# lucanest/Phyloformer

Measured on AMD Instinct MI355X. Metric: alignments/sec, 60-leaf/500-site LG+GC-like MSAs, Phyloformer forward (pf.ckpt), higher is better.
Workload: dtype f16x3-split MFMA (two fp16 limbs per operand, 3 passes), fp32 accumulate/residual

## Files before the change

phyloformer_amd/csrc/pf_device.hip.h:

```cpp
#pragma once
#include <hip/hip_runtime.h>
#include <stdint.h>

#include "pf_layout.h"

namespace pfk {

typedef float f32x4 __attribute__((ext_vector_type(4)));
typedef float f32x16 __attribute__((ext_vector_type(16)));
#if PF_F16
typedef _Float16 h16_t;
#define PF_MFMA(a, b, c) __builtin_amdgcn_mfma_f32_32x32x16_f16((a), (b), (c), 0, 0, 0)
#define PF_DOT2C "v_dot2c_f32_f16"
#define PF_CVT_PK "v_cvt_pk_f16_f32"
#define PF_NEG1_LO 0x0000bc00u
#define PF_NEG1_HI 0xbc000000u
#else
typedef __bf16 h16_t;
#define PF_MFMA(a, b, c) __builtin_amdgcn_mfma_f32_32x32x16_bf16((a), (b), (c), 0, 0, 0)
#define PF_DOT2C "v_dot2c_f32_bf16"
#define PF_CVT_PK "v_cvt_pk_bf16_f32"
#define PF_NEG1_LO 0x0000bf80u
#define PF_NEG1_HI 0xbf800000u
#endif
// ... 1084 lines not shown
        for (int q = 0; q < 8; ++q) v[q] = k + q < nparts ? sp[k + q] : 0.f;
#pragma unroll
        for (int q = 0; q < 8; ++q) acc += v[q];
    }
    out[pr] = acc * (wst ? wst[(size_t)(pr / P) * 4 + 1] : inv_L_total);
}

__global__ void __launch_bounds__(64) k_main_plan(const int* ucount, int* plan, int B, int P, int Lloc, int mode) {
    const int lane = threadIdx.x;
    int* const flist = plan + 4;
    int* const slist = flist + B;
    int* const cpre = slist + B;
    int nf = 0, ns = 0, tiles = 0;
    for (int b0 = 0; b0 < B; b0 += 64) {
        const int b = b0 + lane;
        const int K = b < B ? ucount[b] : 0;
        const bool split = b < B && main_dedup_split(K, Lloc, mode);
        const bool fused = b < B && !split;
        const unsigned long long ms = __ballot(split), mf = __ballot(fused), below = (1ull << lane) - 1ull;
        int incl = split ? compact_tiles(P, K) : 0;
        const int mine = incl;
#pragma unroll
        for (int d = 1; d < 64; d <<= 1) { const int o = __shfl_up(incl, d); if (lane >= d) incl += o; }
        if (split) { const int i = ns + __popcll(ms & below); slist[i] = b; cpre[i] = tiles + incl - mine; }
        if (fused) flist[nf + __popcll(mf & below)] = b;
        ns += __popcll(ms);
        nf += __popcll(mf);
        tiles += __shfl(incl, 63);
    }
    if (lane == 0) { plan[0] = nf; plan[1] = ns; plan[2] = tiles; plan[3] = 0; cpre[ns] = tiles; }
}

template <bool FLAT>
__global__ void __launch_bounds__(256) k_head_parts(MainArgs a) {
    const int ns = *a.acount;
    if (ns == 0) return;
    const int lane = threadIdx.x & 63, t = lane & 31;
    const int ntiles = (a.Lloc + 31) >> 5;
    const int ntasks = ns * a.nt_aln;
    for (int task = blockIdx.x * 4 + (threadIdx.x >> 6); task < ntasks; task += gridDim.x * 4) {
        const TilePos cur = tile_pos<FLAT, ROUTE_LIST>(a, task, ntiles);
        const LanePos lp = lane_pos<FLAT, ROUTE_LIST>(a, cur, t);
        const size_t row0 = ((size_t)cur.b * a.P + cur.r0 + (lp.in_r1 ? 1 : 0)) * a.Lloc;
        const float spz = a.term[row0 + a.srep[(size_t)cur.b * a.Lloc + lp.l]];
        const bool straddle = lp.wrap < 32;
        const long slot0 = (long)cur.b * a.slots_aln + cur.kt + (FLAT ? cur.r0 : 0);
        for (int part = 0; part < (straddle ? 2 : 1); ++part) {
            const float so = half32_sum((lp.valid && lp.in_r1 == (part == 1)) ? spz : 0.f);
            if (lane == 0) a.outpart[slot0 + part] = so;
        }
    }
}

struct SiteClassArgs {
    const uint8_t* idx;
    int* srep;
    int* ulist;
    int* ucount;
    int N, Lloc, dedup;
};
constexpr int SC_THREADS = 1024, SC_MAX_SITES = 4096;
__global__ void __launch_bounds__(SC_THREADS) k_site_classes(SiteClassArgs a) {
    __shared__ __attribute__((aligned(16))) uint32_t hsh[SC_MAX_SITES];
    __shared__ int wsum[SC_THREADS / 64];
    const int b = blockIdx.x, tid = threadIdx.x, lane = tid & 63, wave = tid >> 6;
    const uint8_t* ib = a.idx + (size_t)b * a.N * a.Lloc;
    int* const srep = a.srep + (size_t)b * a.Lloc;
    int* const ulist = a.ulist + (size_t)b * a.Lloc;
    const bool dedup = a.dedup && a.Lloc <= SC_MAX_SITES;
    auto same_column = [&](int c, int l) {
        unsigned diff = 0;
#pragma unroll 8
        for (int n = 0; n < a.N; ++n) diff |= (unsigned)(ib[(size_t)n * a.Lloc + c] ^ ib[(size_t)n * a.Lloc + l]);
        return diff == 0;
    };
    if (dedup) {
        for (int l = tid; l < a.Lloc; l += SC_THREADS) {
            uint32_t hv = 0x811C9DC5u;
#pragma unroll 8
            for (int n = 0; n < a.N; ++n) hv = (hv ^ ib[(size_t)n * a.Lloc + l]) * 0x01000193u;
            hsh[l] = hv;
        }
        __syncthreads();
    }
    int base = 0;
    for (int l0 = 0; l0 < a.Lloc; l0 += SC_THREADS) {
        const int l = l0 + tid;
        int rep = l;
        if (dedup && l < a.Lloc) {
            const uint32_t mine = hsh[l];
            int cand = l;
            for (int c0 = 0; c0 < l && cand == l; c0 += 4) {
                const u32x4 v = *reinterpret_cast<const u32x4*>(hsh + c0);
#pragma unroll
                for (int i = 3; i >= 0; --i)
                    if (v[i] == mine && c0 + i < l) cand = c0 + i;
            }
            if (cand < l) {
                if (same_column(cand, l)) rep = cand;
                else
                    for (int c = cand + 1; c < l && rep == l; ++c)
                        if (hsh[c] == mine && same_column(c, l)) rep = c;
            }
        }
        const bool first = l < a.Lloc && rep == l;
        if (l < a.Lloc) srep[l] = rep;
        const unsigned long long m = __ballot(first);
        if (lane == 0) wsum[wave] = __popcll(m);
        __syncthreads();
        int before = 0, total = 0;
#pragma unroll
        for (int w = 0; w < SC_THREADS / 64; ++w) { const int n = wsum[w]; total += n; if (w < wave) before += n; }
        if (first) ulist[base + before + __popcll(m & ((1ull << lane) - 1ull))] = l;
        base += total;
// ... 434 lines not shown
```

phyloformer_amd/csrc/pf_layout.h:

```cpp
#pragma once

#ifndef PF_F16
#define PF_F16 1
#endif

namespace pfk {

constexpr int E = 64;
constexpr int NH = 4;
constexpr int HD = 16;
constexpr int FF = 256;
constexpr int NA = 22;
constexpr int SROW = 72;
constexpr int MROW = 4 * 64;
constexpr float LN_EPS = 1e-5f;

constexpr int FRAG_W1 = 0;
constexpr int FRAG_W2 = FRAG_W1 + 8 * 4 * 2 * 64;
constexpr int FRAG_WO = FRAG_W2 + 2 * 16 * 2 * 64;
constexpr int FRAG_WV = FRAG_WO + 2 * 4 * 2 * 64;
constexpr int FRAG_QK = FRAG_WV + 2 * 4 * 64;
#ifndef PF_WVLO_LDS
#define PF_WVLO_LDS 4
#endif
constexpr int WVLO_LDS = PF_WVLO_LDS;
constexpr int FRAG_WVLO = FRAG_QK + 4 * 2 * 16;
constexpr int FRAG_END = FRAG_WVLO + WVLO_LDS * 64;
constexpr int FRAG_U = FRAG_WV;
constexpr int U_FRAGS = FF * 4 / 16;
static_assert(FRAG_U + U_FRAGS <= FRAG_END, "the folded head fits the last block's tail");
constexpr int WVLO_FRAGS = 2 * 4 * 64;
constexpr int CONST_B1 = 0, CONST_B2 = 256, CONST_BQK = 320, CONST_HW = 328, CONST_HB = 392,
              CONST_C0 = 393, CONST_BOC = 400;
constexpr int CONST_LEN = 464;
constexpr int MAIN_LDS_BYTES = FRAG_END * 16 + CONST_LEN * 4;
constexpr int MFRAG_PER_PAIR = 2 * 2 * 32;

constexpr int MAIN_THREADS = 512;
constexpr int MAIN_WAVES = MAIN_THREADS / 64;

constexpr int PAIRTAB_ROWS = 22 * 22, PAIRTAB_W = 72;

#if defined(__HIPCC__)
#define PF_HD __host__ __device__
#else
#define PF_HD
#endif
#ifndef PF_MAIN_DEDUP_NUM
#define PF_MAIN_DEDUP_NUM 17
#define PF_MAIN_DEDUP_DEN 20
#endif
constexpr int MAIN_DEDUP_NUM = PF_MAIN_DEDUP_NUM, MAIN_DEDUP_DEN = PF_MAIN_DEDUP_DEN;
PF_HD inline bool main_dedup_split(int K, int L, int mode) {
    return mode == 2 || (mode == 1 && (long)K * MAIN_DEDUP_DEN <= (long)L * MAIN_DEDUP_NUM);
}
PF_HD inline int compact_tiles(int P, int K) { return K >= 32 ? (int)(((long)P * K + 31) >> 5) : P; }
PF_HD inline int compact_nvalid(int P, int K, int kt) {
    const long left = K >= 32 ? (long)P * K - (long)kt * 32 : K;
    return left < 32 ? (int)left : 32;
}
PF_HD inline int compact_wrap(int P, int K, int r0, int u0) {
    return (K >= 32 && r0 + 1 < P && K - u0 < 32) ? K - u0 : 32;
}
struct CompactTile { int r0, u0, nvalid, wrap; };
PF_HD inline CompactTile compact_tile(int P, int K, int kt) {
    CompactTile c;
    if (K >= 32) { const long tok0 = (long)kt * 32; c.r0 = (int)(tok0 / K); c.u0 = (int)(tok0 - (long)c.r0 * K); }
    else { c.r0 = kt; c.u0 = 0; }
    c.nvalid = compact_nvalid(P, K, kt);
    c.wrap = compact_wrap(P, K, c.r0, c.u0);
    return c;
}
PF_HD inline void compact_next(int K, int* r0, int* u0) {
    if (K < 32) { ++*r0; return; }
    *u0 += 32;
    if (*u0 >= K) { *u0 -= K; ++*r0; }
}
PF_HD inline int main_plan_ints(int B) { return 4 + 3 * B + 1; }

}
```

phyloformer_amd/csrc/pf_lib.hip:

```cpp
#include <hip/hip_runtime.h>
#include <dlfcn.h>

#include <algorithm>
#include <cmath>
#include <cstdarg>
#include <cstdio>
#include <cstdlib>
#include <cstring>
#include <functional>
#include <map>
#include <mutex>
#include <string>
#include <type_traits>
#include <vector>

#include "../../include/phyloformer_amd.h"
#include "pf_device.hip.h"
#include "pf_mha.hip.h"
#include "pf_precise.hip.h"
#include "pf_generic.hip.h"
#include "pf_boot.hip.h"
#include "pf_sites.hip.h"
#include "pf_sitemap.hip.h"
#include "pf_sites_host.h"
// ... 119 lines not shown
    std::vector<pfp::FfnW> ffn;
};

struct GenericWeights {
    F64Ends ends;
    bool ready = false;
    std::vector<pfg::AttnW> row, col;
    std::vector<pfg::FfnW> ffn;
};

constexpr int64_t SUB_FLOATS_DEFAULT = (int64_t)1 << 22;

struct DeviceBuffer {
    void* p = nullptr; size_t cap = 0;
    explicit DeviceBuffer(std::vector<DeviceBuffer*>& all) { all.push_back(this); }
    DeviceBuffer(const DeviceBuffer&) = delete;
    int reserve(pf_handle* h, size_t bytes);
    void release() { if (p) hipFree(p); p = nullptr; cap = 0; }
};
template <class T> struct Buffer : DeviceBuffer {
    using DeviceBuffer::DeviceBuffer;
    operator T*() const { return static_cast<T*>(p); }
};

}

struct pf_handle {
    int device = 0;
    int n_blocks = 0;
    hipStream_t stream = nullptr;
    hipStream_t stream2 = nullptr;
    hipStream_t cur = nullptr;
    hipEvent_t ev_fork = nullptr, ev_join = nullptr;
    hipDeviceProp_t prop;
    std::string err;
    int64_t max_seqs = 200;
    bool profile = false;
    bool profile_main_only = false;
    bool debug_keep = false;
    int ablate = 0;
    unsigned long long* phase_prof = nullptr;
    bool phase_prof_last = false;
    bool head_fold = true;
    bool force_rccl = false;
    int64_t ws_limit_bytes = (int64_t)24 << 30;
    float* table = nullptr;
    float* pair_table = nullptr;
    bool embed_mfma = false;
    int colstats_fine = -1;
    bool colstats_ring = true;
    bool materialize_x0 = false;
    bool site_dedup = true;
    int main_dedup = 1;
    float* first_consts = nullptr;
    float* first_img = nullptr;
    std::vector<BlockDev> blk;
    std::vector<void*> owned;
    std::vector<DeviceBuffer*> buffers;
    int pair_n = -1;
    Buffer<int16_t> pair_i{buffers}, pair_j{buffers};
    Buffer<char> ws{buffers}, ws2{buffers};
    bool overlap = true;
    int reserve_cus = 8;
    Buffer<uint8_t> d_idx{buffers};
    Buffer<float> d_out{buffers};
    Buffer<uint8_t> d_rep{buffers};
    Buffer<int32_t> d_map{buffers};
    Buffer<float> d_smap{buffers}, d_se{buffers}, d_prof{buffers};
    Buffer<double> d_mpart{buffers};
    Buffer<char> d_sub{buffers};
    int64_t sub_floats = SUB_FLOATS_DEFAULT;
    pftile::Plan tiled_plan;
    pftile::Tables tiled_tab;
    Buffer<char> d_tiled_tab{buffers};
    Buffer<char> d_nj{buffers}, d_nj_io{buffers};
    int64_t nj_calls = 0;
    int64_t bionj_calls = 0;
    Buffer<char> d_delta_io{buffers};
    int64_t delta_calls = 0;
    bool delta_atomic = true;
    Buffer<char> d_fit{buffers}, d_fit_io{buffers};
    int64_t fit_calls = 0;
    int64_t fit_lds_bytes = pffit::LDS_MAX_BYTES;
    Buffer<char> d_ols{buffers}, d_ols_io{buffers};
    int64_t ols_calls = 0;
    Buffer<char> d_bme{buffers};
    Buffer<float> d_bme_preds{buffers};
    int64_t bme_calls = 0;
    int64_t spr_calls = 0;
    bool spr_pairs_simple = false;
    int64_t spr_step_cap = 0;
    Buffer<char> d_sup{buffers}, d_sup_io{buffers};
    Buffer<uint8_t> d_sup_bad{buffers};
    int64_t sup_calls = 0;
    int64_t transfer_calls = 0;
    Buffer<char> d_con{buffers}, d_con_io{buffers};
    int64_t con_calls = 0;
    Buffer<char> d_td{buffers}, d_td_io{buffers};
    int64_t td_calls = 0;
    Buffer<float> d_w{buffers}, d_wst{buffers}, d_wtab{buffers};
    void* comm[2] = {nullptr, nullptr};
    int rank = 0, world = 1;
    int64_t coll_calls = 0;
    bool sharded_call = false;
    bool reducing = false;
    bool two_streams = true;
// ... 291 lines not shown
int save_tap(pf_handle* h, const std::string& name, const float* dptr, size_t n) {
    std::vector<float>& v = h->taps[name];
    v.resize(n);
    HIPCHK(h, hipStreamSynchronize(h->cur));
    HIPCHK(h, hipMemcpy(v.data(), dptr, n * sizeof(float), hipMemcpyDeviceToHost));
    return PF_OK;
}

int allreduce(pf_handle* h, void* buf, size_t count, int dtype = NCCL_FLOAT) {
    if (!h->sharded_call) return PF_OK;
    if (h->world <= 1 && !h->comm[0]) return PF_OK;
    if (!h->comm[0]) return fail(h, PF_ESTATE, "sharded forward on %d ranks needs pf_comm_init", h->world);
    ProfScope ps(h, K_ALLREDUCE);
    void* comm = h->comm[(h->cur == h->stream2 && h->stream2) ? 1 : 0];
    ++h->coll_calls;
    int rc = g_rccl.AllReduce(buf, buf, count, dtype, NCCL_SUM, comm, h->cur);
    if (rc != 0)
        return fail(h, PF_ERCCL, "ncclAllReduce failed: %s",
                    g_rccl.GetErrorString ? g_rccl.GetErrorString(rc) : "?");
    return PF_OK;
}

enum { PLAIN = 0, SITEMAP = 1, WEIGHTED = 2 };
constexpr int HEAD_PARTS = MODE_STATS + 1;
struct MainKind { int mode, flavour = PLAIN, route = ROUTE_ALL; };
using MainKernel = void (*)(MainArgs);
struct MainRow { MainKind kind; bool flat; MainKernel fn; };
const std::vector<MainRow>& main_kernels();

MainKernel main_kernel(MainKind k, bool flat) {
    for (const MainRow& r : main_kernels())
        if (r.kind.mode == k.mode && r.kind.flavour == k.flavour && r.kind.route == k.route && r.flat == flat) return r.fn;
    return nullptr;
}

int persistent_grid(const pf_handle* h, long ntasks, int per_block, int per_cu) {
    const int cus = std::max(1, h->prop.multiProcessorCount - (h->reducing ? h->reserve_cus : 0));
    return (int)std::max<long>(1, std::min<long>((long)per_cu * cus, (ntasks + per_block - 1) / per_block));
}

int launch_main(pf_handle* h, MainKind kind, const MainArgs& a, bool timed) {
    const MainKernel fn = main_kernel(kind, kind.route == ROUTE_COMPACT || a.flat);
    if (!fn) return fail(h, PF_ESTATE, "no k_main for mode %d, flavour %d, route %d", kind.mode, kind.flavour, kind.route);
    const int grid = persistent_grid(h, (long)a.B * a.nt_aln, MAIN_WAVES, 1);
    ProfScope ps(h, kind.mode == MODE_FIRST ? K_EMBED : K_MAIN, timed);
    hipLaunchKernelGGL(fn, dim3(grid), dim3(MAIN_THREADS), MAIN_LDS_BYTES, h->cur, a);
    HIPCHK(h, hipGetLastError());
    return PF_OK;
}

struct MainPlan { const int *nf, *ns, *flist, *slist, *cpre; };
MainPlan main_plan(const int* plan, int B) { return {&plan[0], &plan[1], &plan[4], &plan[4 + B], &plan[4 + 2 * B]}; }

int launch_main_routed(pf_handle* h, int mode, const MainArgs& m, const MainPlan& p) {
    int rc;
    MainArgs f = m, c = m;
    f.acount = p.nf; f.alist = p.flist;
    if ((rc = launch_main(h, {mode, PLAIN, ROUTE_LIST}, f, false))) return rc;
    c.acount = p.ns; c.alist = p.slist; c.cpre = p.cpre;
    c.term = m.spart; c.prof = nullptr;
    if ((rc = launch_main(h, {mode, PLAIN, ROUTE_COMPACT}, c, false))) return rc;
    if (mode != MODE_LAST && mode != MODE_LAST_FOLD) return launch_main(h, {MODE_STATS, PLAIN, ROUTE_LIST}, c, false);
    hipLaunchKernelGGL(main_kernel({HEAD_PARTS, PLAIN, ROUTE_LIST}, m.flat != 0), dim3(persistent_grid(h, (long)m.B * m.nt_aln, 4, 8)),
                       dim3(256), 0, h->cur, c);
    HIPCHK(h, hipGetLastError());
    return PF_OK;
}

struct RowStats { const float* p; int nparts; int flat; };
struct ShardRun {
    Workspace w;
    const uint8_t* d_idx;
    float* d_out;
    int B, N, P, Lloc, L_total;
    TilePlan tp;
    hipStream_t stream;
    RowStats rs;
    float* d_smap = nullptr;
    const float* d_w = nullptr;
    const float* d_wst = nullptr;
    bool routed = false;
};

int zero_fill(pf_handle* h, float* p, size_t n) {
    HIPCHK(h, hipMemsetAsync(p, 0, n * sizeof(float), h->cur));
    return PF_OK;
}

MainArgs main_args(pf_handle* h, const ShardRun& r) {
    MainArgs m{};
    m.x = r.w.x; m.qrow = r.w.qrow; m.qcol = r.w.qcol;
    m.mfrag = reinterpret_cast<const frag_t*>(r.w.mfrag); m.rq = r.w.rq; m.ctx = r.w.ctx; m.spart = r.w.spart;
    m.outpart = r.w.outpart; m.table = h->table; m.idx = r.d_idx; m.pair_i = h->pair_i; m.pair_j = h->pair_j;
    m.B = r.B; m.N = r.N; m.P = r.P; m.Lloc = r.Lloc;
    m.flat = r.tp.flat; m.nt_aln = r.tp.nt_aln; m.slots_aln = r.tp.slots_aln;
    m.store_x_last = h->debug_keep ? 1 : 0;
    m.trash_tok = (size_t)r.B * r.P * r.Lloc;
    m.ablate = h->ablate;
    m.prof = h->phase_prof_last ? nullptr : h->phase_prof;
    m.w = r.d_w;
    m.srep = r.w.srep;
    m.ulist = r.w.ulist; m.ucount = r.w.ucount;
    return m;
}

bool x0_on_the_fly(const pf_handle* h) {
    return !h->materialize_x0 && !h->embed_mfma && h->n_blocks > 1;
}

bool routes_main(const pf_handle* h, const ShardRun& r) {
    return h->main_dedup != 0 && !r.d_smap && !r.d_w && x0_on_the_fly(h) && r.Lloc > 0;
}

ShardRun shard_run(const pf_handle* h, const uint8_t* d_idx, float* d_out, int B, int N, int Lloc, int L_total,
                   float* d_smap = nullptr, const float* d_w = nullptr, const float* d_wst = nullptr) {
    ShardRun r{};
    r.d_idx = d_idx; r.d_out = d_out; r.d_smap = d_smap; r.d_w = d_w; r.d_wst = d_wst;
    r.B = B; r.N = N; r.P = N * (N - 1) / 2; r.Lloc = Lloc; r.L_total = L_total;
    r.tp = tile_plan(h, r.P, Lloc); r.stream = h->stream; r.routed = routes_main(h, r);
    return r;
}

int launch_site_classes(pf_handle* h, const SiteClassArgs& a, int B, int* plan = nullptr, int P = 0) {
    if (!a.Lloc) return PF_OK;
    ProfScope ps(h, K_SITE_CLASSES);
    hipLaunchKernelGGL(k_site_classes, dim3(B), dim3(SC_THREADS), 0, h->cur, a);
    HIPCHK(h, hipGetLastError());
    if (!plan) return PF_OK;
    hipLaunchKernelGGL(k_main_plan, dim3(1), dim3(64), 0, h->cur, a.ucount, plan, B, P, a.Lloc, h->main_dedup);
    HIPCHK(h, hipGetLastError());
    return PF_OK;
}

int save_route_taps(pf_handle* h, const ShardRun& r) {
    if (!r.Lloc) return PF_OK;
    const size_t nsite = (size_t)r.B * r.Lloc;
    int rc;
    if ((rc = save_tap(h, "srep", reinterpret_cast<const float*>(r.w.srep), nsite))) return rc;
    if ((rc = save_tap(h, "ulist", reinterpret_cast<const float*>(r.w.ulist), nsite))) return rc;
    if ((rc = save_tap(h, "ucount", reinterpret_cast<const float*>(r.w.ucount), (size_t)r.B))) return rc;
    if (r.routed) return save_tap(h, "plan", reinterpret_cast<const float*>(r.w.plan), (size_t)main_plan_ints(r.B));
    h->taps.erase("plan");
    return PF_OK;
}

int phase_first(pf_handle* h, const ShardRun& r) {
    if (!r.Lloc) return zero_fill(h, r.w.srow, (size_t)r.B * r.P * SROW);
    int rc;
    if (h->embed_mfma) {
        MainArgs m = main_args(h, r);
        m.wimg = reinterpret_cast<const frag_t*>(h->first_img); m.consts = h->first_consts;
        m.wv_lo = reinterpret_cast<const frag_t*>(h->blk[0].wv_lo);
        if ((rc = launch_main(h, {MODE_FIRST}, m, true))) return rc;
    } else {
        float* x0 = (x0_on_the_fly(h) && !h->debug_keep) ? nullptr : r.w.x;
        EmbedArgs e{r.d_idx, h->pair_i, h->pair_j, h->pair_table, h->table, x0, r.w.qrow, r.w.srow,
                    r.B, r.N, r.P, r.Lloc, h->bad_idx_dev, r.d_w};
        const int ntasks = r.B * r.P, wpb = EMBED_THREADS / 64;
        const int grid = std::max(1, std::min(h->prop.multiProcessorCount, (ntasks + wpb - 1) / wpb));
        ProfScope ps(h, K_EMBED);
        if (r.d_w) hipLaunchKernelGGL(k_embed<true>, dim3(grid), dim3(EMBED_THREADS), EMBED_LDS_BYTES, h->cur, e);
        else hipLaunchKernelGGL(k_embed<false>, dim3(grid), dim3(EMBED_THREADS), EMBED_LDS_BYTES, h->cur, e);
        HIPCHK(h, hipGetLastError());
    }
    if (h->debug_keep) return save_tap(h, "x0", r.w.x, (size_t)r.B * r.P * r.Lloc * 64);
    return PF_OK;
}

int tiles_of(int Lloc) { return (Lloc + 31) / 32; }

int launch_rowsum(pf_handle* h, const ShardRun& r, RowStats* rs) {
    if (rs->p == r.w.srow) return PF_OK;
    const int n = r.B * r.P * SROW;
    if (!r.Lloc) { *rs = RowStats{r.w.srow, 1, 0}; return zero_fill(h, r.w.srow, n); }
    ProfScope ps(h, K_ROWFIN);
    hipLaunchKernelGGL(k_rowsum, dim3((n + 255) / 256), dim3(256), 0, h->cur, rs->p, r.w.srow, r.B * r.P, rs->nparts,
                       rs->flat, r.P, r.Lloc, r.tp.slots_aln);
    HIPCHK(h, hipGetLastError());
    *rs = RowStats{r.w.srow, 1, 0};
    return PF_OK;
}

// ... 55 lines not shown
template <int MODE, bool FLAT, int FLAVOUR = PLAIN, int ROUTE = ROUTE_ALL>
MainRow main_row() { return {{MODE, FLAVOUR, ROUTE}, FLAT, k_main<MODE, FLAT, FLAVOUR == SITEMAP, FLAVOUR == WEIGHTED, ROUTE>}; }
template <bool FLAT>
MainRow head_parts_row() { return {{HEAD_PARTS, PLAIN, ROUTE_LIST}, FLAT, k_head_parts<FLAT>}; }
const std::vector<MainRow>& main_kernels() {
    static const std::vector<MainRow> rows = {
        main_row<MODE_MID0, true, PLAIN, ROUTE_LIST>(), main_row<MODE_MID0, false, PLAIN, ROUTE_LIST>(), main_row<MODE_MID0, true, PLAIN, ROUTE_COMPACT>(),
        main_row<MODE_STATS, true, PLAIN, ROUTE_LIST>(), main_row<MODE_STATS, false, PLAIN, ROUTE_LIST>(), head_parts_row<true>(), head_parts_row<false>(),
        main_row<MODE_MID, true, PLAIN, ROUTE_LIST>(), main_row<MODE_MID, false, PLAIN, ROUTE_LIST>(), main_row<MODE_MID, true, PLAIN, ROUTE_COMPACT>(),
        main_row<MODE_LAST, true, PLAIN, ROUTE_LIST>(), main_row<MODE_LAST, false, PLAIN, ROUTE_LIST>(), main_row<MODE_LAST, true, PLAIN, ROUTE_COMPACT>(),
        main_row<MODE_LAST_FOLD, true, PLAIN, ROUTE_LIST>(), main_row<MODE_LAST_FOLD, false, PLAIN, ROUTE_LIST>(), main_row<MODE_LAST_FOLD, true, PLAIN, ROUTE_COMPACT>(),
        main_row<MODE_FIRST, false>(), main_row<MODE_MID, false>(), main_row<MODE_MID0, false>(), main_row<MODE_LAST, false>(), main_row<MODE_LAST_FOLD, false>(),
        main_row<MODE_FIRST, true>(), main_row<MODE_MID, true>(), main_row<MODE_MID0, true>(), main_row<MODE_LAST, true>(), main_row<MODE_LAST_FOLD, true>(),
        main_row<MODE_LAST, false, SITEMAP>(), main_row<MODE_LAST_FOLD, false, SITEMAP>(), main_row<MODE_LAST, true, SITEMAP>(), main_row<MODE_LAST_FOLD, true, SITEMAP>(),
        main_row<MODE_MID, false, WEIGHTED>(), main_row<MODE_MID0, false, WEIGHTED>(), main_row<MODE_LAST, false, WEIGHTED>(), main_row<MODE_LAST_FOLD, false, WEIGHTED>(),
        main_row<MODE_MID, true, WEIGHTED>(), main_row<MODE_MID0, true, WEIGHTED>(), main_row<MODE_LAST, true, WEIGHTED>(), main_row<MODE_LAST_FOLD, true, WEIGHTED>(),
    };
    return rows;
}

struct BlockKind { MainKind kind; bool routed; };
BlockKind block_kind(const pf_handle* h, const ShardRun& r, int k) {
    const bool last = k + 1 >= h->n_blocks;
    const MainKind kind{!last ? (k == 0 && x0_on_the_fly(h) ? MODE_MID0 : MODE_MID) : (h->head_fold ? MODE_LAST_FOLD : MODE_LAST),
                        r.d_w ? WEIGHTED : (r.d_smap && last) ? SITEMAP : PLAIN};
    return {kind, r.routed && !(kind.mode == MODE_LAST && h->debug_keep)};
}

int launch_block_main(pf_handle* h, const ShardRun& r, int k) {
    const BlockKind b = block_kind(h, r, k);
    const bool last = k + 1 >= h->n_blocks;
    MainArgs m = main_args(h, r);
    m.wimg = reinterpret_cast<const frag_t*>(h->blk[k].wimg); m.consts = h->blk[k].consts;
    m.wv_lo = last ? nullptr : reinterpret_cast<const frag_t*>(h->blk[k + 1].wv_lo);
    if (last) { m.sitemap = r.d_smap; if (h->phase_prof_last) m.prof = h->phase_prof; }
    ProfScope ps(h, K_MAIN, r.routed);
    int rc = b.routed ? launch_main_routed(h, b.kind.mode, m, main_plan(r.w.plan, r.B)) : launch_main(h, b.kind, m, !r.routed);
    if (rc || b.kind.mode != MODE_LAST_FOLD || !h->debug_keep) return rc;
    m.outpart = r.w.spart; m.prof = nullptr;
    return launch_main(h, {MODE_LAST, r.d_w ? WEIGHTED : PLAIN}, m, !r.routed);
}

int phase_block(pf_handle* h, const ShardRun& r, int k, RowStats rs) {
    if (!r.Lloc) return PF_OK;
    const std::string tag = std::to_string(k);
    const size_t pairs = (size_t)r.B * r.P, sites = (size_t)r.B * r.Lloc;
    int rc;
    if (h->debug_keep && ((rc = launch_rowsum(h, r, &rs)) || (rc = save_tap(h, "srow" + tag, rs.p, pairs * SROW)))) return rc;
    if ((rc = launch_rowfin(h, r, k, rs))) return rc;
    if ((rc = launch_colstats(h, r, k))) return rc;
    if ((rc = launch_colfin(h, r, k))) return rc;
    if (h->debug_keep && ((rc = save_tap(h, "ctx" + tag, r.w.ctx, sites * 64)) || (rc = save_tap(h, "mrow" + tag, r.w.mrow, pairs * MROW)))) return rc;
    if ((rc = launch_block_main(h, r, k))) return rc;
    if (h->debug_keep) return save_tap(h, "x" + std::to_string(k + 1), r.w.x, pairs * r.Lloc * 64);
    return PF_OK;
}

bool reduces_now(const pf_handle* h) { return h->sharded_call && (h->world > 1 || h->comm[0]); }
bool empty_rank_call(const pf_handle* h, int Lloc) { return Lloc == 0 && reduces_now(h); }

int halves_of(const pf_handle* h, int B) {
    if (B < 2 || h->debug_keep) return 1;
    if (reduces_now(h)) return h->overlap ? 2 : 1;
    return h->two_streams ? 2 : 1;
}

int ensure_second_stream(pf_handle* h) {
    if (h->stream2) return PF_OK;
    HIPCHK(h, hipStreamCreateWithFlags(&h->stream2, hipStreamNonBlocking));
    HIPCHK(h, hipEventCreateWithFlags(&h->ev_fork, hipEventDisableTiming));
    HIPCHK(h, hipEventCreateWithFlags(&h->ev_join, hipEventDisableTiming));
    return PF_OK;
}

struct ForwardScope {
    pf_handle* h;
    ForwardScope(pf_handle* h_, bool reduces) : h(h_) { h->reducing = reduces; }
    ~ForwardScope() { h->cur = h->stream; h->reducing = false; }
};

template <class Reduce>
int schedule(pf_handle* h, ShardRun* runs, size_t nruns, Reduce reduce) {
    ShardRun* const end = runs + nruns;
    int rc;
    for (ShardRun* r = runs; r != end; ++r) {
        h->cur = r->stream;
        const SiteClassArgs sc{r->d_idx, r->w.srep, r->w.ulist, r->w.ucount, r->N, r->Lloc, h->site_dedup ? 1 : 0};
        if ((rc = launch_site_classes(h, sc, r->B, r->routed ? r->w.plan : nullptr, r->P))) return rc;
        if (h->debug_keep && (rc = save_route_taps(h, *r))) return rc;
        if ((rc = phase_first(h, *r))) return rc;
        r->rs = first_stats(h, *r);
    }
    for (int k = 0; k < h->n_blocks; ++k) {
        if ((rc = reduce(false))) return rc;
        for (ShardRun* r = runs; r != end; ++r) {
            h->cur = r->stream;
            if ((rc = phase_block(h, *r, k, r->rs))) return rc;
            r->rs = main_stats(*r);
        }
    }
    for (ShardRun* r = runs; r != end; ++r) {
        h->cur = r->stream;
        if ((rc = launch_outsum(h, *r))) return rc;
    }
    return reduce(true);
}

int forward_chunk(pf_handle* h, const uint8_t* d_idx, int B, int N, int Lloc, int L_total, float* d_out,
                  float* d_smap = nullptr, const float* d_w = nullptr, const float* d_wst = nullptr) {
    const int P = N * (N - 1) / 2;
    const bool reduces = reduces_now(h);
    const int nh = halves_of(h, B);
    int rc = ensure_pairs(h, N);
    if (rc) return rc;
    ShardRun r[2]{};
    int b0 = 0;
    for (int i = 0; i < nh; ++i) {
        const int nb = (nh == 2) ? (i == 0 ? (B + 1) / 2 : B / 2) : B;
        r[i] = shard_run(h, d_idx + (size_t)b0 * N * Lloc, d_out + (size_t)b0 * P, nb, N, Lloc, L_total,
                         d_smap ? d_smap + (size_t)b0 * P * Lloc : nullptr, d_w ? d_w + (size_t)b0 * Lloc : nullptr,
                         d_w ? d_wst + (size_t)b0 * pfw::WST : nullptr);
        if ((rc = ensure_workspace(h, nb, P, Lloc, &r[i].w, i == 1))) return rc;
        b0 += nb;
    }
    ForwardScope scope(h, reduces);
    if (nh == 2) {
        if ((rc = ensure_second_stream(h))) return rc;
        r[1].stream = h->stream2;
        HIPCHK(h, hipEventRecord(h->ev_fork, h->stream));
        HIPCHK(h, hipStreamWaitEvent(h->stream2, h->ev_fork, 0));
    }
    auto reduce = [&](bool site_sums) -> int {
        if (!reduces) return PF_OK;
        for (ShardRun* q = r; q != r + nh; ++q) {
            h->cur = q->stream;
            if (!site_sums && (rc = launch_rowsum(h, *q, &q->rs))) return rc;
            if ((rc = allreduce(h, site_sums ? q->d_out : q->w.srow, (size_t)q->B * P * (site_sums ? 1 : SROW)))) return rc;
        }
        return PF_OK;
    };
    if ((rc = schedule(h, r, nh, reduce))) return rc;
// ... 1412 lines not shown
    int rc2 = plan_distances(h, B, K, N, &nb);
    if (rc2 || (!device && (rc2 = check_join_tables(h, nullptr, user.slots, user.flag, B, K, N)))) return rc2;
    HIPCHK(h, hipSetDevice(h->device));
    ++h->td_calls;
    if (device) return distances_launch(h, user, B, K, N, nb);
    return staged_call(h, h->d_td_io, list, [&] { return distances_launch(h, io, B, K, N, nb); });
}

}

extern "C" {

int pf_abi_version(void) { return PF_ABI_VERSION; }

uint64_t pf_blob_len(int32_t n_blocks, int32_t n_heads, int32_t embed_dim) {
    return read_blob(nullptr, n_blocks, embed_dim, n_heads).len;
}

static int open_device(int device, pf_handle** out) {
    int ndev = 0;
    hipError_t e = hipGetDeviceCount(&ndev);
    if (e != hipSuccess || ndev == 0)
        return fail(nullptr, PF_EHIP, "no HIP device available (%s); there is no CPU fallback",
                    e != hipSuccess ? hipGetErrorString(e) : "device count is 0");
    if (device < 0 || device >= ndev) return fail(nullptr, PF_EINVAL, "device %d out of range (have %d)", device, ndev);
    pf_handle* h = new pf_handle();
    if (const char* e = getenv("PF_TWO_STREAMS")) h->two_streams = atoi(e) != 0;
    if (getenv("PF_ROW_TILES")) h->tile_force = 0;
    if (getenv("PF_FLAT_TILES")) h->tile_force = 1;
    if (const char* v = getenv("PF_COLSTATS_RING")) h->colstats_ring = atoi(v) != 0;
    h->device = device;
    int rc = PF_OK;
    do {
        if ((e = hipSetDevice(device)) != hipSuccess) { rc = fail(nullptr, PF_EHIP, "hipSetDevice: %s", hipGetErrorString(e)); break; }
        if ((e = hipGetDeviceProperties(&h->prop, device)) != hipSuccess) { rc = fail(nullptr, PF_EHIP, "hipGetDeviceProperties: %s", hipGetErrorString(e)); break; }
        if (std::string(h->prop.gcnArchName).rfind("gfx950", 0) != 0) {
            rc = fail(nullptr, PF_EHIP, "device %d is %s; this library is built for gfx950 only", device, h->prop.gcnArchName);
            break;
        }
        if ((e = hipStreamCreateWithFlags(&h->stream, hipStreamNonBlocking)) != hipSuccess) { rc = fail(nullptr, PF_EHIP, "hipStreamCreate: %s", hipGetErrorString(e)); break; }
        h->cur = h->stream;
        if ((e = hipHostMalloc((void**)&h->bad_idx_host, 3 * sizeof(unsigned), hipHostMallocMapped | hipHostMallocCoherent)) != hipSuccess ||
            (e = hipHostGetDevicePointer((void**)&h->bad_idx_dev, h->bad_idx_host, 0)) != hipSuccess) {
            rc = fail(nullptr, PF_EHIP, "hipHostMalloc (residue flag): %s", hipGetErrorString(e));
            break;
        }
        h->bad_idx_host[0] = h->bad_idx_host[1] = h->bad_idx_host[2] = 0u;
        auto big_lds = [&](const void* fn, int bytes) {
            if (!rc && (e = hipFuncSetAttribute(fn, hipFuncAttributeMaxDynamicSharedMemorySize, bytes)) != hipSuccess)
                rc = fail(nullptr, PF_EHIP, "hipFuncSetAttribute: %s", hipGetErrorString(e));
        };
        for (const MainRow& r : main_kernels())
            if (r.kind.route == ROUTE_ALL) big_lds(reinterpret_cast<const void*>(r.fn), MAIN_LDS_BYTES);
        big_lds(reinterpret_cast<const void*>(&k_embed<false>), EMBED_LDS_BYTES);
        big_lds(reinterpret_cast<const void*>(&k_embed<true>), EMBED_LDS_BYTES);
        big_lds(reinterpret_cast<const void*>(&pffit::k_fit_setup), pffit::SETUP_LDS_MAX);
        big_lds(reinterpret_cast<const void*>(&pffit::k_fit_pairs<true>), pffit::LDS_MAX_BYTES);
        big_lds(reinterpret_cast<const void*>(&pfols::k_ols_setup), pfols::SETUP_LDS_MAX);
        if (rc) break;
    } while (0);
    if (rc) { pf_destroy(h); return rc; }
    *out = h;
    return PF_OK;
}

int pf_create_bare(int device, pf_handle_t** out) {
    if (!out) return fail(nullptr, PF_EINVAL, "null argument");
    *out = nullptr;
    return open_device(device, out);
}

int pf_create(const pf_weights_t* w, int device, pf_handle_t** out) {
    if (!w || !out || !w->blob) return fail(nullptr, PF_EINVAL, "null argument");
    *out = nullptr;
    if (!generic_arch_ok(w))
        return fail(nullptr, PF_EINVAL,
                    "unsupported architecture: n_blocks=%d n_heads=%d embed_dim=%d n_alphabet=%d "
                    "(n_alphabet must be 22, n_blocks 1..64, embed_dim must be 1..256 and divisible by n_heads)",
                    w->n_blocks, w->n_heads, w->embed_dim, w->n_alphabet);
    if (w->blob_len != pf_blob_len(w->n_blocks, w->n_heads, w->embed_dim))
        return fail(nullptr, PF_EINVAL, "weight blob has %llu floats, expected %llu",
                    (unsigned long long)w->blob_len,
                    (unsigned long long)pf_blob_len(w->n_blocks, w->n_heads, w->embed_dim));
    pf_handle* h = nullptr;
    int rc = open_device(device, &h);
    if (rc) return rc;
    h->n_blocks = w->n_blocks;
    h->garch = pfg::make_arch(w->embed_dim, w->n_heads);
    const BlobView bv = read_blob(w->blob, w->n_blocks, w->embed_dim, w->n_heads);
    if (w->embed_dim == E && w->n_heads == NH) {
        rc = prepare_weights(h, bv, w->blob_len);
        if (!rc) rc = prepare_precise_weights(h, bv, &h->pw);
        if (!rc) {
            try { h->blob_copy.assign(w->blob, w->blob + w->blob_len); }
            catch (const std::bad_alloc&) { rc = fail(h, PF_ENOMEM, "out of host memory copying the weights"); }
        }
    } else {
        h->arch_generic = true;
        rc = prepare_generic_weights(h, bv);
    }
    if (rc) g_create_error = h->err;
    if (rc) { pf_destroy(h); return rc; }
    *out = h;
    return PF_OK;
}

int pf_destroy(pf_handle_t* h) {
    if (!h) return PF_OK;
    hipSetDevice(h->device);
    if (h->stream) hipStreamSynchronize(h->stream);
    if (h->stream2) hipStreamSynchronize(h->stream2);
    for (void*& c : h->comm) if (c && g_rccl.CommDestroy) { g_rccl.CommDestroy(c); c = nullptr; }
    for (auto& s : h->pending) { hipEventDestroy(s.a); hipEventDestroy(s.b); }
    for (auto e : h->free_events) hipEventDestroy(e);
    for (void* p : h->owned) hipFree(p);
    for (DeviceBuffer* b : h->buffers) b->release();
    if (h->stream2) hipStreamDestroy(h->stream2);
    if (h->ev_fork) hipEventDestroy(h->ev_fork);
    if (h->ev_join) hipEventDestroy(h->ev_join);
    if (h->stream) hipStreamDestroy(h->stream);
    if (h->bad_idx_host) hipHostFree(h->bad_idx_host);
    delete h;
    return PF_OK;
}

const char* pf_last_error(const pf_handle_t* h) { return h ? h->err.c_str() : g_create_error.c_str(); }

int pf_set_option(pf_handle_t* h, const char* key, int64_t value) {
    if (!h || !key) return PF_EINVAL;
    const std::string k(key);
    if (k == "max_seqs") h->max_seqs = value;
    else if (k == "profile") { drain_profile(h); h->profile = value != 0; h->profile_main_only = value == 2; }
    else if (k == "debug_keep") h->debug_keep = value != 0;
    else if (k == "embed_mfma") h->embed_mfma = value != 0;
    else if (k == "colstats_fine") h->colstats_fine = value < 0 ? -1 : (value != 0);
    else if (k == "materialize_x0") h->materialize_x0 = value != 0;
    else if (k == "overlap") h->overlap = value != 0;
    else if (k == "two_streams") h->two_streams = value != 0;
    else if (k == "reserve_cus") h->reserve_cus = (int)std::max<int64_t>(0, std::min<int64_t>(value, 128));
    else if (k == "ablate") h->ablate = (int)value;
    else if (k == "head_fold") h->head_fold = value != 0;
    else if (k == "force_rccl") h->force_rccl = value != 0;
    else if (k == "colstats_ring") h->colstats_ring = value != 0;
    else if (k == "site_dedup") h->site_dedup = value != 0;
    else if (k == "main_dedup") h->main_dedup = value <= 0 ? 0 : (value >= 2 ? 2 : 1);
    else if (k == "precise") h->precise = value < 0 ? -1 : (value != 0);
    else if (k == "recheck_above") h->recheck_above = value > 0 ? (double)value : 0.0;
    else if (k == "precise_ffn_valu") h->precise_ffn_valu = value != 0;
    else if (k == "generic") {
        if (h->arch_generic && !value)
            return fail(h, PF_EINVAL, "embed_dim %d / n_heads %d runs on the generic kernels only (option generic cannot be 0)",
                        h->garch.E, h->garch.NH);
        h->generic = value != 0;
    }
    else if (k == "phase_prof") {
        if (value && !h->phase_prof) { HIPCHK(h, hipMalloc((void**)&h->phase_prof, 64)); h->owned.push_back(h->phase_prof); }
        if (h->phase_prof) HIPCHK(h, hipMemset(h->phase_prof, 0, 64));
        if (!value) h->phase_prof = nullptr;
        h->phase_prof_last = value == 2;
    }
    else if (k == "ws_limit_mb") h->ws_limit_bytes = value << 20;
    else if (k == "spr_pairs_simple") h->spr_pairs_simple = value != 0;
    else if (k == "delta_atomic") h->delta_atomic = value != 0;
    else if (k == "fit_lds_bytes") h->fit_lds_bytes = value > 0 ? std::min<int64_t>(value, pffit::LDS_MAX_BYTES) : pffit::LDS_MAX_BYTES;
    else if (k == "spr_step_cap") h->spr_step_cap = value > 0 ? value : 0;
    else if (k == "sub_floats") h->sub_floats = value > 0 ? value : SUB_FLOATS_DEFAULT;
    else return fail(h, PF_EINVAL, "unknown option '%s'", key);
    return PF_OK;
}

int pf_forward(pf_handle_t* h, const uint8_t* idx, int32_t B, int32_t N, int32_t L, float* out) {
    if (!h) return PF_EINVAL;
    return forward_host_impl(h, idx, B, N, 0, L, L, out);
}

int pf_resample_sites_device(pf_handle_t* h, const uint8_t* d_src, int32_t B, int32_t N, int32_t L, int32_t r_begin, int32_t R,
                             uint64_t seed, uint8_t* d_dst) {
    if (!h) return PF_EINVAL;
    if (!d_src || !d_dst) return fail(h, PF_EINVAL, "null buffer");
    if (B < 1 || N < 1 || L < 1 || R < 1 || r_begin < 0)
        return fail(h, PF_EINVAL, "bad dimensions B=%d N=%d L=%d r_begin=%d R=%d", B, N, L, r_begin, R);
    size_t n = 0;
    if (!mul_size((size_t)B, (size_t)R, (size_t)N * L, &n))
        return fail(h, PF_EINVAL, "B=%d x R=%d replicates of %d x %d overflow the address space", B, R, N, L);
    HIPCHK(h, hipSetDevice(h->device));
    return launch_resample(h, d_src, B, N, L, r_begin, R, seed, d_dst);
}

int pf_bootstrap(pf_handle_t* h, const uint8_t* idx, int32_t B, int32_t N, int32_t L, int32_t R, uint64_t seed, float* out) {
    if (!h) return PF_EINVAL;
    return bootstrap_impl(h, idx, B, N, L, R, seed, out);
}

int pf_window_count(int32_t L, int32_t W, int32_t step) {
    const int n = pfsites::window_count(L, W, step);
    return n < 0 ? PF_EINVAL : n;
}

// ... 784 lines not shown
```

Baseline: 659.5.

## Compute split-route attention stats once per unique site column via row kernel

Adds a persistent k_row_stats kernel for dedup-routed alignments. For each row it computes the LayerNorm, QK and V projections only for unique site columns, caches the results in an LDS term table, and then reduces per-tile key/value stats by mapping each site back to its representative. Repeated sites are filled into x with a separate copy kernel, and alignments whose unique count exceeds the LDS capacity fall back to the old stats launch through a device-built big list. This avoids redundant MFMA work on duplicated columns, at the cost of extra launches, LDS pressure and a serial search in find().

```diff
diff --git a/phyloformer_amd/csrc/pf_device.hip.h b/phyloformer_amd/csrc/pf_device.hip.h
--- a/phyloformer_amd/csrc/pf_device.hip.h
+++ b/phyloformer_amd/csrc/pf_device.hip.h
@@ -1160,6 +1160,201 @@
     }
 }
 
+constexpr int ROW_STATS_THREADS = MAIN_THREADS, ROW_STATS_WAVES = ROW_STATS_THREADS / 64;
+struct RowItem { int b, p, K; bool ok; };
+__global__ void __launch_bounds__(64) k_stats_plan(const int* ucount, const int* plan, int* big, int B) {
+    const int lane = threadIdx.x, ns = plan[1];
+    const int* const slist = plan + 4 + B;
+    int nb = 0;
+    for (int i0 = 0; i0 < ns; i0 += 64) {
+        const int b = i0 + lane < ns ? slist[i0 + lane] : 0;
+        const bool is_big = i0 + lane < ns && ucount[b] > ROW_STATS_KMAX;
+        const unsigned long long m = __ballot(is_big);
+        if (is_big) big[1 + nb + __popcll(m & ((1ull << lane) - 1ull))] = b;
+        nb += __popcll(m);
+    }
+    if (lane == 0) big[0] = nb;
+}
+
+__global__ void __launch_bounds__(256) k_copy_repeats(MainArgs a) {
+    const int ns = *a.acount;
+    const size_t per = (size_t)a.P * a.Lloc * 16, n = (size_t)ns * per;
+    for (size_t i = (size_t)blockIdx.x * blockDim.x + threadIdx.x; i < n; i += (size_t)gridDim.x * blockDim.x) {
+        const int b = a.alist[i / per];
+        if (a.ucount[b] > ROW_STATS_KMAX) continue;
+        const size_t r = i % per, tok = r >> 4;
+        const int l = (int)(tok % a.Lloc), rep = a.srep[(size_t)b * a.Lloc + l];
+        if (rep == l) continue;
+        f32x4* const xa = reinterpret_cast<f32x4*>(a.x + (size_t)b * a.P * a.Lloc * 64);
+        xa[(tok * 16) + (r & 15)] = xa[((tok - l + rep) * 16) + (r & 15)];
+    }
+}
+
+__global__ void __launch_bounds__(ROW_STATS_THREADS, ROW_STATS_WAVES / 4) k_row_stats(MainArgs a) {
+    extern __shared__ __attribute__((aligned(16))) unsigned char smem[];
+    const int ns = *a.acount;
+    if (ns == 0) return;
+    int sj = 0, seen = 0;
+    RowItem hit{0, 0, 0, false};
+    auto find = [&](int item) {
+        RowItem it{0, 0, 0, false};
+        const int qi = item / a.P;
+        if (hit.ok && seen == qi) { it = hit; it.p = item - qi * a.P; return it; }
+        for (; sj < ns; ++sj) {
+            const int b = a.alist[sj], K = a.ucount[b];
+            if (K > ROW_STATS_KMAX) continue;
+            if (seen == qi) { it.b = b; it.p = item - qi * a.P; it.K = K; it.ok = true; hit = it; return it; }
+            ++seen;
+        }
+        hit.ok = false;
+        return it;
+    };
+    int item = blockIdx.x;
+    RowItem cur = find(item);
+    if (!cur.ok) return;
+
+    const int lane = threadIdx.x & 63;
+    const int wave = __builtin_amdgcn_readfirstlane(threadIdx.x >> 6);
+    const int t = lane & 31, h = lane >> 5;
+    const int L = a.Lloc;
+    unsigned short* const map = reinterpret_cast<unsigned short*>(smem + ROW_STATS_OFF_MAP);
+    float* const bqk = reinterpret_cast<float*>(smem + ROW_STATS_OFF_BQK);
+    float* const term = reinterpret_cast<float*>(smem + ROW_STATS_OFF_TERM);
+    auto build_map = [&](int b, int K) {
+        const int* const ul = a.ulist + (size_t)b * L;
+        const int* const sr = a.srep + (size_t)b * L;
+        for (int u = threadIdx.x; u < K; u += ROW_STATS_THREADS) map[ul[u]] = (unsigned short)u;
+        __syncthreads();
+        for (int l = threadIdx.x; l < L; l += ROW_STATS_THREADS) { const int r = sr[l]; if (r != l) map[l] = map[r]; }
+    };
+    f32x4 px[8];
+    auto prefetch = [&](const RowItem& it, int ct) {
+        const int u = min(32 * ct + t, it.K - 1);
+        const int l = a.ulist[(size_t)it.b * L + u];
+        const f32x4* xp = reinterpret_cast<const f32x4*>(a.x + (((size_t)it.b * a.P + it.p) * L + l) * 64 + 4 * h);
+#pragma unroll
+        for (int g = 0; g < 8; ++g) px[g] = xp[2 * g];
+    };
+    prefetch(cur, wave);
+    {
+        frag_t* const lf = reinterpret_cast<frag_t*>(smem);
+        const frag_t* const img = a.wimg + FRAG_WV;
+        for (int f = threadIdx.x; f < ROW_STATS_FRAG_WVLO; f += ROW_STATS_THREADS) lf[f] = img[f];
+        for (int f = threadIdx.x; f < WVLO_FRAGS; f += ROW_STATS_THREADS) lf[ROW_STATS_FRAG_WVLO + f] = a.wv_lo[f];
+        if (threadIdx.x < 8) bqk[threadIdx.x] = a.consts[CONST_BQK + threadIdx.x];
+        static_assert(FRAG_QK - FRAG_WV == ROW_STATS_FRAG_QK && FRAG_WVLO - FRAG_QK == ROW_STATS_FRAG_WVLO - ROW_STATS_FRAG_QK, "one copy");
+    }
+    build_map(cur.b, cur.K);
+    __syncthreads();
+
+    lds_frag_t lw = (lds_frag_t)smem;
+    lds_frag_t qkp = lw + ROW_STATS_FRAG_QK + h * 8 + (t & 7);
+    lds_frag_t wvp = lw + ROW_STATS_FRAG_WV + lane;
+    lds_f32_t lbq = (lds_f32_t)(smem + ROW_STATS_OFF_BQK) + 4 * h;
+    PF_OPAQUE(qkp); PF_OPAQUE(wvp);
+
+    for (;;) {
+        const int b = cur.b, p = cur.p, K = cur.K;
+        const int nct = row_ctiles(K);
+        item += gridDim.x;
+        const RowItem nxt = find(item);
+        for (int ct = wave;; ct += ROW_STATS_WAVES) {
+            float x[32];
+#pragma unroll
+            for (int g = 0; g < 8; ++g)
+#pragma unroll
+                for (int i = 0; i < 4; ++i) x[4 * g + i] = px[g][i];
+            const bool more = ct + ROW_STATS_WAVES < nct;
+            prefetch(more || !nxt.ok ? cur : nxt, more ? ct + ROW_STATS_WAVES : wave);
+            if (ct >= nct) break;
+            f32x16 va[3];
+            {
+                float xn[32];
+                ln_pair(x, xn);
+                frag_t xb_hi[4], xb_lo[4];
+#pragma unroll
+                for (int s = 0; s < 4; ++s) split8(&xn[8 * s], xb_hi[s], xb_lo[s]);
+#pragma unroll
+                for (int s = 0; s < 4; ++s) {
+                    const frag_t q_hi = qkp[(s * 2) * 16], q_lo = qkp[(s * 2 + 1) * 16];
+                    if (s == 0) mfma3_zero(va[2], q_hi, q_lo, xb_hi[s], xb_lo[s]);
+                    else mfma3(va[2], q_hi, q_lo, xb_hi[s], xb_lo[s]);
+                }
+#pragma unroll
+                for (int s = 0; s < 4; ++s)
+#pragma unroll
+                    for (int T = 0; T < 2; ++T) {
+                        const frag_t f_hi = wvp[(T * 4 + s) * 64];
+                        const frag_t f_lo = wvp[(ROW_STATS_FRAG_WVLO - ROW_STATS_FRAG_WV) + (T * 4 + s) * 64];
+                        if (s == 0) mfma3_zero(va[T], f_hi, f_lo, xb_hi[s], xb_lo[s], T == 1);
+                        else mfma3(va[T], f_hi, f_lo, xb_hi[s], xb_lo[s], T == 1);
+                    }
+            }
+#pragma unroll
+            for (int r = 0; r < 4; ++r) va[2][r] += lbq[r];
+            float qk[4];
+#pragma unroll
+            for (int i = 0; i < 4; ++i) qk[i] = elu1_fast(va[2][i]);
+            const int u = 32 * ct + t;
+            if (u < K) {
+                f32x4* const tr = reinterpret_cast<f32x4*>(term + (size_t)u * ROW_STATS_TERM);
+#pragma unroll
+                for (int g = 0; g < 8; ++g) {
+                    const f32x4 v4 = {va[g >> 2][4 * (g & 3)], va[g >> 2][4 * (g & 3) + 1], va[g >> 2][4 * (g & 3) + 2], va[g >> 2][4 * (g & 3) + 3]};
+                    tr[8 * h + g] = v4;
+                }
+                const f32x4 own = {qk[0], qk[1], qk[2], qk[3]};
+                tr[16 + h] = own;
+            }
+            if (!more) break;
+        }
+        __syncthreads();
+
+        const int nparts = row_parts(a.flat, L, p);
+        for (int j = wave; j < nparts; j += ROW_STATS_WAVES) {
+            const RowPart rp = row_part(a.flat, L, p, j);
+            const int l = rp.l0 + t;
+            const bool valid = l >= 0 && l < L;
+            const int lc_ = min(max(l, 0), L - 1);
+            const f32x4* const tr = reinterpret_cast<const f32x4*>(term + (size_t)map[lc_] * ROW_STATS_TERM);
+            float vv[32];
+#pragma unroll
+            for (int g = 0; g < 8; ++g) {
+                const f32x4 v4 = tr[8 * h + g];
+#pragma unroll
+                for (int i = 0; i < 4; ++i) vv[4 * g + i] = v4[i];
+            }
+            const f32x4 q4 = tr[16], k4 = tr[17];
+            const float qn[4] = {q4[0], q4[1], q4[2], q4[3]}, kn[4] = {k4[0], k4[1], k4[2], k4[3]};
+            if (valid && h == 0) {
+                *reinterpret_cast<f32x4*>(a.qrow + (((size_t)b * a.P + p) * L + l) * 4) = q4;
+            }
+            float* sp = a.spart + (size_t)((long)b * a.slots_aln + rp.slot) * SROW;
+            const float vm = valid ? 1.f : 0.f;
+            float km[4];
+#pragma unroll
+            for (int i = 0; i < 4; ++i) km[i] = kn[i] * vm;
+            {
+                float qk8[8];
+#pragma unroll
+                for (int i = 0; i < 4; ++i) { qk8[i] = vm * qn[i]; qk8[4 + i] = km[i]; }
+                const float sqk = treduce8(qk8, t);
+                if (lane < 8) sp[64 + lane] = sqk;
+            }
+            {
+                float kv[32];
+#pragma unroll
+                for (int jj = 0; jj < 32; ++jj) kv[jj] = valid ? km[jj >> 3] * vv[jj] : 0.f;
+                sp[kmap(t, h)] = treduce32(kv, t);
+            }
+        }
+        if (!nxt.ok) break;
+        __syncthreads();
+        if (nxt.b != b) { build_map(nxt.b, nxt.K); }
+        cur = nxt;
+    }
+}
+
 struct SiteClassArgs {
     const uint8_t* idx;
     int* srep;
@@ -1168,6 +1363,8 @@
     int N, Lloc, dedup;
 };
 constexpr int SC_THREADS = 1024, SC_MAX_SITES = 4096;
+static_assert(SC_MAX_SITES <= ROW_STATS_MAP_SITES && ROW_STATS_KMAX <= SC_MAX_SITES,
+              "k_row_stats' site map holds every alignment with K <= ROW_STATS_KMAX < L (beyond SC_MAX_SITES: K = L)");
 __global__ void __launch_bounds__(SC_THREADS) k_site_classes(SiteClassArgs a) {
     __shared__ __attribute__((aligned(16))) uint32_t hsh[SC_MAX_SITES];
     __shared__ int wsum[SC_THREADS / 64];
diff --git a/phyloformer_amd/csrc/pf_layout.h b/phyloformer_amd/csrc/pf_layout.h
--- a/phyloformer_amd/csrc/pf_layout.h
+++ b/phyloformer_amd/csrc/pf_layout.h
@@ -54,6 +54,9 @@
 PF_HD inline bool main_dedup_split(int K, int L, int mode) {
     return mode == 2 || (mode == 1 && (long)K * MAIN_DEDUP_DEN <= (long)L * MAIN_DEDUP_NUM);
 }
+PF_HD inline int main_dedup_max_k(int L, int mode) {
+    return mode == 2 ? L : mode == 1 ? (int)((long)L * MAIN_DEDUP_NUM / MAIN_DEDUP_DEN) : 0;
+}
 PF_HD inline int compact_tiles(int P, int K) { return K >= 32 ? (int)(((long)P * K + 31) >> 5) : P; }
 PF_HD inline int compact_nvalid(int P, int K, int kt) {
     const long left = K >= 32 ? (long)P * K - (long)kt * 32 : K;
@@ -78,4 +81,34 @@
 }
 PF_HD inline int main_plan_ints(int B) { return 4 + 3 * B + 1; }
 
+constexpr int ROW_STATS_FRAG_WV = 0;
+constexpr int ROW_STATS_FRAG_QK = ROW_STATS_FRAG_WV + 2 * 4 * 64;
+constexpr int ROW_STATS_FRAG_WVLO = ROW_STATS_FRAG_QK + 4 * 2 * 16;
+constexpr int ROW_STATS_FRAGS = ROW_STATS_FRAG_WVLO + WVLO_FRAGS;
+constexpr int ROW_STATS_MAP_SITES = 4096;
+constexpr int ROW_STATS_TERM = 76;
+constexpr int ROW_STATS_OFF_BQK = ROW_STATS_FRAGS * 16;
+constexpr int ROW_STATS_OFF_MAP = ROW_STATS_OFF_BQK + 8 * 4;
+constexpr int ROW_STATS_OFF_TERM = ROW_STATS_OFF_MAP + ROW_STATS_MAP_SITES * 2;
+constexpr int ROW_STATS_KMAX = 451;
+static_assert(ROW_STATS_KMAX == (160 * 1024 - ROW_STATS_OFF_TERM) / (ROW_STATS_TERM * 4), "KMAX is derived from the LDS left");
+constexpr int ROW_STATS_LDS_BYTES = ROW_STATS_OFF_TERM + ROW_STATS_KMAX * ROW_STATS_TERM * 4;
+static_assert(ROW_STATS_KMAX >= 425, "every split-route alignment of 500 sites (K <= 17 / 20 L) fits the term table");
+static_assert(ROW_STATS_OFF_TERM % 16 == 0 && ROW_STATS_LDS_BYTES <= 160 * 1024, "the term table is read 16 bytes at a time");
+PF_HD inline int row_ctiles(int K) { return (K + 31) >> 5; }
+PF_HD inline int row_ctile_nvalid(int K, int ct) { return K - 32 * ct < 32 ? K - 32 * ct : 32; }
+struct RowPart { int kt, l0, slot; };
+PF_HD inline int row_parts(int flat, int L, int p) {
+    if (!flat) return (L + 31) >> 5;
+    return (int)(((((long)p + 1) * L - 1) >> 5) - (((long)p * L) >> 5)) + 1;
 }
+PF_HD inline RowPart row_part(int flat, int L, int p, int j) {
+    RowPart r;
+    if (!flat) { r.kt = p * ((L + 31) >> 5) + j; r.l0 = 32 * j; r.slot = r.kt; return r; }
+    r.kt = (int)(((long)p * L) >> 5) + j;
+    r.l0 = (int)((long)r.kt * 32 - (long)p * L);
+    r.slot = r.kt + p;
+    return r;
+}
+
+}
diff --git a/phyloformer_amd/csrc/pf_lib.hip b/phyloformer_amd/csrc/pf_lib.hip
--- a/phyloformer_amd/csrc/pf_lib.hip
+++ b/phyloformer_amd/csrc/pf_lib.hip
@@ -195,6 +195,7 @@
     bool materialize_x0 = false;
     bool site_dedup = true;
     int main_dedup = 1;
+    bool stats_dedup = true;
     float* first_consts = nullptr;
     float* first_img = nullptr;
     std::vector<BlockDev> blk;
@@ -592,6 +593,28 @@
 struct MainPlan { const int *nf, *ns, *flist, *slist, *cpre; };
 MainPlan main_plan(const int* plan, int B) { return {&plan[0], &plan[1], &plan[4], &plan[4 + B], &plan[4 + 2 * B]}; }
 
+enum { STATS_ROWS, STATS_ROWS_BIG, STATS_LAUNCH };
+int split_stats_form(const pf_handle* h, int Lloc) {
+    if (!h->stats_dedup || Lloc > ROW_STATS_MAP_SITES) return STATS_LAUNCH;
+    return std::min(Lloc, main_dedup_max_k(Lloc, h->main_dedup)) <= ROW_STATS_KMAX ? STATS_ROWS : STATS_ROWS_BIG;
+}
+int* stats_big_list(float* outpart) { return reinterpret_cast<int*>(outpart); }
+
+int launch_split_stats(pf_handle* h, const MainArgs& c) {
+    const int form = split_stats_form(h, c.Lloc);
+    if (form == STATS_LAUNCH) return launch_main(h, {MODE_STATS, PLAIN, ROUTE_LIST}, c, false);
+    hipLaunchKernelGGL(k_row_stats, dim3(persistent_grid(h, (long)c.B * c.P, 1, 1)), dim3(ROW_STATS_THREADS), ROW_STATS_LDS_BYTES, h->cur, c);
+    HIPCHK(h, hipGetLastError());
+    if (c.store_x_last) {
+        hipLaunchKernelGGL(k_copy_repeats, dim3(persistent_grid(h, (long)c.B * c.P * c.Lloc * 16, 256, 8)), dim3(256), 0, h->cur, c);
+        HIPCHK(h, hipGetLastError());
+    }
+    if (form == STATS_ROWS) return PF_OK;
+    MainArgs s = c;
+    s.acount = stats_big_list(c.outpart); s.alist = s.acount + 1;
+    return launch_main(h, {MODE_STATS, PLAIN, ROUTE_LIST}, s, false);
+}
+
 int launch_main_routed(pf_handle* h, int mode, const MainArgs& m, const MainPlan& p) {
     int rc;
     MainArgs f = m, c = m;
@@ -600,7 +623,7 @@
     c.acount = p.ns; c.alist = p.slist; c.cpre = p.cpre;
     c.term = m.spart; c.prof = nullptr;
     if ((rc = launch_main(h, {mode, PLAIN, ROUTE_COMPACT}, c, false))) return rc;
-    if (mode != MODE_LAST && mode != MODE_LAST_FOLD) return launch_main(h, {MODE_STATS, PLAIN, ROUTE_LIST}, c, false);
+    if (mode != MODE_LAST && mode != MODE_LAST_FOLD) return launch_split_stats(h, c);
     hipLaunchKernelGGL(main_kernel({HEAD_PARTS, PLAIN, ROUTE_LIST}, m.flat != 0), dim3(persistent_grid(h, (long)m.B * m.nt_aln, 4, 8)),
                        dim3(256), 0, h->cur, c);
     HIPCHK(h, hipGetLastError());
@@ -661,13 +684,16 @@
     return r;
 }
 
-int launch_site_classes(pf_handle* h, const SiteClassArgs& a, int B, int* plan = nullptr, int P = 0) {
+int launch_site_classes(pf_handle* h, const SiteClassArgs& a, int B, int* plan = nullptr, int P = 0, int* stats_big = nullptr) {
     if (!a.Lloc) return PF_OK;
     ProfScope ps(h, K_SITE_CLASSES);
     hipLaunchKernelGGL(k_site_classes, dim3(B), dim3(SC_THREADS), 0, h->cur, a);
     HIPCHK(h, hipGetLastError());
     if (!plan) return PF_OK;
     hipLaunchKernelGGL(k_main_plan, dim3(1), dim3(64), 0, h->cur, a.ucount, plan, B, P, a.Lloc, h->main_dedup);
+    HIPCHK(h, hipGetLastError());
+    if (!stats_big) return PF_OK;
+    hipLaunchKernelGGL(k_stats_plan, dim3(1), dim3(64), 0, h->cur, a.ucount, plan, stats_big, B);
     HIPCHK(h, hipGetLastError());
     return PF_OK;
 }
@@ -829,6 +855,7 @@
     if ((rc = launch_colfin(h, r, k))) return rc;
     if (h->debug_keep && ((rc = save_tap(h, "ctx" + tag, r.w.ctx, sites * 64)) || (rc = save_tap(h, "mrow" + tag, r.w.mrow, pairs * MROW)))) return rc;
     if ((rc = launch_block_main(h, r, k))) return rc;
+    if (h->debug_keep && k + 1 < h->n_blocks && (rc = save_tap(h, "qrow" + std::to_string(k + 1), r.w.qrow, pairs * r.Lloc * 4))) return rc;
     if (h->debug_keep) return save_tap(h, "x" + std::to_string(k + 1), r.w.x, pairs * r.Lloc * 64);
     return PF_OK;
 }
@@ -863,7 +890,8 @@
     for (ShardRun* r = runs; r != end; ++r) {
         h->cur = r->stream;
         const SiteClassArgs sc{r->d_idx, r->w.srep, r->w.ulist, r->w.ucount, r->N, r->Lloc, h->site_dedup ? 1 : 0};
-        if ((rc = launch_site_classes(h, sc, r->B, r->routed ? r->w.plan : nullptr, r->P))) return rc;
+        int* const big = r->routed && split_stats_form(h, r->Lloc) == STATS_ROWS_BIG ? stats_big_list(r->w.outpart) : nullptr;
+        if ((rc = launch_site_classes(h, sc, r->B, r->routed ? r->w.plan : nullptr, r->P, big))) return rc;
         if (h->debug_keep && (rc = save_route_taps(h, *r))) return rc;
         if ((rc = phase_first(h, *r))) return rc;
         r->rs = first_stats(h, *r);
@@ -2382,6 +2410,7 @@
         };
         for (const MainRow& r : main_kernels())
             if (r.kind.route == ROUTE_ALL) big_lds(reinterpret_cast<const void*>(r.fn), MAIN_LDS_BYTES);
+        big_lds(reinterpret_cast<const void*>(&k_row_stats), ROW_STATS_LDS_BYTES);
         big_lds(reinterpret_cast<const void*>(&k_embed<false>), EMBED_LDS_BYTES);
         big_lds(reinterpret_cast<const void*>(&k_embed<true>), EMBED_LDS_BYTES);
         big_lds(reinterpret_cast<const void*>(&pffit::k_fit_setup), pffit::SETUP_LDS_MAX);
@@ -2474,6 +2503,7 @@
     else if (k == "colstats_ring") h->colstats_ring = value != 0;
     else if (k == "site_dedup") h->site_dedup = value != 0;
     else if (k == "main_dedup") h->main_dedup = value <= 0 ? 0 : (value >= 2 ? 2 : 1);
+    else if (k == "stats_dedup") h->stats_dedup = value != 0;
     else if (k == "precise") h->precise = value < 0 ? -1 : (value != 0);
     else if (k == "recheck_above") h->recheck_above = value > 0 ? (double)value : 0.0;
     else if (k == "precise_ffn_valu") h->precise_ffn_valu = value != 0;
```

After: 673.7, median of 6. 1.02x the previous value.
